# HKUST-KnowComp/DummyNode4GraphLearning

Hardware: AMD Instinct MI355X
Metric: edges/sec fwd+bwd on dummy-augmented RGIN conv (higher is better)
Workload: dtype bf16; 1 GPU; config5: RGINLayer(256,256,R=16,basis,relu) fwd+bwd, ONE global batch of 32768 graphs cut by parallel.shard_graphs over 1 GPU(s) (rank 0: N=1015808, E=3997696), SI dummy augmentation; global_edges=3997696, parallelism=dp1, rows_P=3112960, grad_bucket_bytes=2491904, hip_graph=True, sub_batches=1

## Files before the change

### dummynode4graphlearning_amd/csrc/dn_chain_wgrad.hip

```cpp
#include "dn_common.h"
#include "dn_internal.h"
#include "../../include/dn_hip.h"

namespace {

constexpr int kH = 256;
constexpr int kTile = 64;
constexpr int kKC = 32;
constexpr int kThreads = 256;
constexpr int kAld = kTile + 2;

__device__ __forceinline__ double bf16_to_f64(bf16_t v) { return (double)(float)v; }

__device__ __forceinline__ bf16_t f64_to_bf16(double d) {
    float f = (float)d;
    if ((double)f != d && f == f && fabsf(f) < __builtin_huge_valf()) {
        uint32_t u = __float_as_uint(f);
        if (fabs((double)f) > fabs(d)) u -= 1u;
        f = __uint_as_float(u | 1u);
    }
    return (bf16_t)f;
}

__global__ __launch_bounds__(kThreads) void chain_combine_products_kernel(const float* __restrict__ M, const bf16_t* __restrict__ W1,
                                                                          const bf16_t* __restrict__ Wc,
                                                                          const bf16_t* __restrict__ Wc_loop, int32_t R,
                                                                          bf16_t* __restrict__ dWc, double* __restrict__ part) {
    __shared__ __attribute__((aligned(16))) double As[kKC * kAld];
    __shared__ __attribute__((aligned(16))) double Bs[kKC * kTile];
    const int tid = threadIdx.x, ty = tid >> 4, tx = tid & 15;
    const int m0 = (int)(blockIdx.x >> 2) * kTile, n0 = (int)(blockIdx.x & 3) * kTile;
    const int r = (int)blockIdx.y, kind = (int)blockIdx.z;
    const float* Mr = M + (size_t)r * kH * kH;
    const bf16_t* B = kind == 0 ? W1 : (r < R ? Wc + (size_t)r * kH * kH : Wc_loop);
    double acc[4][4];
#pragma unroll
    for (int i = 0; i < 4; ++i)
#pragma unroll
        for (int j = 0; j < 4; ++j) acc[i][j] = 0.0;
    float ra[8];
    bf16_t rb[8];
    auto fetch = [&](int kc) __attribute__((always_inline)) {
#pragma unroll
        for (int s = 0; s < 8; ++s) {
            if (kind == 0) ra[s] = Mr[(size_t)(m0 + (tid >> 5) + 8 * s) * kH + kc + (tid & 31)];
            else ra[s] = Mr[(size_t)(kc + (tid >> 6) + 4 * s) * kH + m0 + (tid & 63)];
            rb[s] = B[(size_t)(kc + (tid >> 6) + 4 * s) * kH + n0 + (tid & 63)];
        }
    };
    fetch(0);
    for (int kc = 0; kc < kH; kc += kKC) {
#pragma unroll
        for (int s = 0; s < 8; ++s) {
            if (kind == 0) As[(tid & 31) * kAld + (tid >> 5) + 8 * s] = (double)ra[s];
            else As[((tid >> 6) + 4 * s) * kAld + (tid & 63)] = (double)ra[s];
            Bs[((tid >> 6) + 4 * s) * kTile + (tid & 63)] = bf16_to_f64(rb[s]);
        }
        if (kc + kKC < kH) fetch(kc + kKC);
        __syncthreads();
#pragma unroll 8
        for (int k = 0; k < kKC; ++k) {
            const double2 a01 = *reinterpret_cast<const double2*>(&As[k * kAld + 4 * ty]);
            const double2 a23 = *reinterpret_cast<const double2*>(&As[k * kAld + 4 * ty + 2]);
            const double2 b01 = *reinterpret_cast<const double2*>(&Bs[k * kTile + 4 * tx]);
            const double2 b23 = *reinterpret_cast<const double2*>(&Bs[k * kTile + 4 * tx + 2]);
            const double a[4] = {a01.x, a01.y, a23.x, a23.y}, b[4] = {b01.x, b01.y, b23.x, b23.y};
#pragma unroll
            for (int i = 0; i < 4; ++i)
#pragma unroll
                for (int j = 0; j < 4; ++j) acc[i][j] = fma(a[i], b[j], acc[i][j]);
        }
        __syncthreads();
    }
#pragma unroll
    for (int i = 0; i < 4; ++i)
#pragma unroll
        for (int j = 0; j < 4; ++j) {
            const size_t o = (size_t)r * kH * kH + (size_t)(m0 + 4 * ty + i) * kH + n0 + 4 * tx + j;
            if (kind == 0) dWc[o] = f64_to_bf16(acc[i][j]);
            else part[o] = acc[i][j];
        }
}

__global__ __launch_bounds__(kH) void chain_combine_finish_kernel(const double* __restrict__ part, const float* __restrict__ c,
                                                                  const bf16_t* __restrict__ W1, const bf16_t* __restrict__ bias,
                                                                  int32_t R, bf16_t* __restrict__ dW1, bf16_t* __restrict__ db,
                                                                  bf16_t* __restrict__ db1) {
    const int h = threadIdx.x, j = (int)blockIdx.x;
    if (j < kH) {
        double sum = 0.0;
        for (int r = 0; r <= R; ++r) sum += part[(size_t)r * kH * kH + (size_t)j * kH + h];
        if (bias) sum = fma((double)c[j], bf16_to_f64(bias[h]), sum);
        dW1[(size_t)j * kH + h] = f64_to_bf16(sum);
        return;
    }
    if (db) {
        double sum = 0.0;
        for (int jj = 0; jj < kH; ++jj) sum = fma((double)c[jj], bf16_to_f64(W1[(size_t)jj * kH + h]), sum);
        db[h] = f64_to_bf16(sum);
    }
    if (db1) db1[h] = (bf16_t)c[h];
}

}

extern "C" int dn_layer_chain_dgrad_bf16(const void* G1, const void* W_kn, int64_t N, int32_t H, const int32_t* tiles, int64_t num_tiles,
                                         void* G0, void* seg_sums, dn_stream_t stream) {
    DN_REQUIRE(H == 256, "dn_layer_chain_dgrad: unsupported width %d (256 only)", H);
    DN_REQUIRE(N >= 0 && N < 0x7fffffffLL && num_tiles >= 0 && num_tiles < 0x7fffffffLL, "dn_layer_chain_dgrad: bad sizes");
    if (num_tiles == 0) return DN_OK;
    DN_REQUIRE(G1 && W_kn && tiles && G0 && seg_sums, "dn_layer_chain_dgrad: NULL pointer");
    DN_REQUIRE((reinterpret_cast<uintptr_t>(G1) | reinterpret_cast<uintptr_t>(W_kn) | reinterpret_cast<uintptr_t>(tiles) |
                reinterpret_cast<uintptr_t>(G0) | reinterpret_cast<uintptr_t>(seg_sums)) % 16 == 0, "dn_layer_chain_dgrad: unaligned pointer");
    return dn_internal::launch_transform_ring256_seg(G1, W_kn, tiles, num_tiles, G0, seg_sums, (hipStream_t)stream);
}

extern "C" size_t dn_layer_chain_wgrad_combine_workspace_bytes(int64_t R, int32_t H) {
    return R >= 0 && H > 0 ? (size_t)(R + 1) * (size_t)H * (size_t)H * sizeof(double) : 0;
}

extern "C" int dn_layer_chain_wgrad_combine(const float* M, const float* c, const void* W1, const void* Wc, const void* Wc_loop,
                                            const void* bias, int64_t R, int32_t H, void* dWc, void* db, void* dW1, void* db1,
                                            void* workspace, size_t workspace_bytes, dn_stream_t stream) {
    DN_REQUIRE(H == 256, "dn_layer_chain_wgrad_combine: unsupported width %d (256 only)", H);
    DN_REQUIRE(R >= 0 && R < 65535, "dn_layer_chain_wgrad_combine: bad relation count");
    DN_REQUIRE(M && c && W1 && Wc_loop && dWc && dW1 && workspace && (Wc || R == 0), "dn_layer_chain_wgrad_combine: NULL pointer");
    DN_REQUIRE(workspace_bytes >= dn_layer_chain_wgrad_combine_workspace_bytes(R, H), "dn_layer_chain_wgrad_combine: workspace too small");
    DN_REQUIRE((reinterpret_cast<uintptr_t>(M) | reinterpret_cast<uintptr_t>(workspace)) % 16 == 0,
               "dn_layer_chain_wgrad_combine: unaligned pointer");
    hipStream_t st = (hipStream_t)stream;
    double* part = (double*)workspace;
    hipLaunchKernelGGL(chain_combine_products_kernel, dim3((kH / kTile) * (kH / kTile), (unsigned)(R + 1), 2), dim3(kThreads), 0, st, M,
                       (const bf16_t*)W1, (const bf16_t*)Wc, (const bf16_t*)Wc_loop, (int32_t)R, (bf16_t*)dWc, part);
    DN_CHECK_LAUNCH();
    hipLaunchKernelGGL(chain_combine_finish_kernel, dim3(kH + 1), dim3(kH), 0, st, (const double*)part, c, (const bf16_t*)W1,
                       (const bf16_t*)bias, (int32_t)R, (bf16_t*)dW1, (bf16_t*)db, (bf16_t*)db1);
    DN_CHECK_LAUNCH();
    return DN_OK;
}
```

Baseline: 1.430 billion edges/s.

## Rebalance wgrad combine GEMMs into persistent grid with tail slabs and double buffering

Replaces the per-tile 3D grid of fp64 combine GEMMs with a fixed persistent grid of 256 blocks. Each block runs larger 128x64 tiles, and the leftover tiles are split into small slabs spread across all blocks, so the last wave is not left lopsided. Shared-memory staging is double-buffered with register prefetch. The db/db1 reduction moves into an extra block of the products kernel, and the finish kernel batches its partial-sum loads. The trade-off is more register and LDS pressure per block and more complex scheduling code.

```diff
diff --git a/dummynode4graphlearning_amd/csrc/dn_chain_wgrad.hip b/dummynode4graphlearning_amd/csrc/dn_chain_wgrad.hip
--- a/dummynode4graphlearning_amd/csrc/dn_chain_wgrad.hip
+++ b/dummynode4graphlearning_amd/csrc/dn_chain_wgrad.hip
@@ -5,10 +5,14 @@
 namespace {
 
 constexpr int kH = 256;
-constexpr int kTile = 64;
-constexpr int kKC = 32;
+constexpr int kKC = 16;
+constexpr int kChunks = kH / kKC;
 constexpr int kThreads = 256;
-constexpr int kAld = kTile + 2;
+constexpr int kGrid = 256;
+constexpr int kAPad = 2;
+constexpr int kPartialBatch = 17;
+
+typedef double f64x2 __attribute__((ext_vector_type(2)));
 
 __device__ __forceinline__ double bf16_to_f64(bf16_t v) { return (double)(float)v; }
 
@@ -22,84 +26,212 @@
     return (bf16_t)f;
 }
 
-__global__ __launch_bounds__(kThreads) void chain_combine_products_kernel(const float* __restrict__ M, const bf16_t* __restrict__ W1,
-                                                                          const bf16_t* __restrict__ Wc,
-                                                                          const bf16_t* __restrict__ Wc_loop, int32_t R,
-                                                                          bf16_t* __restrict__ dWc, double* __restrict__ part) {
-    __shared__ __attribute__((aligned(16))) double As[kKC * kAld];
-    __shared__ __attribute__((aligned(16))) double Bs[kKC * kTile];
-    const int tid = threadIdx.x, ty = tid >> 4, tx = tid & 15;
-    const int m0 = (int)(blockIdx.x >> 2) * kTile, n0 = (int)(blockIdx.x & 3) * kTile;
-    const int r = (int)blockIdx.y, kind = (int)blockIdx.z;
-    const float* Mr = M + (size_t)r * kH * kH;
-    const bf16_t* B = kind == 0 ? W1 : (r < R ? Wc + (size_t)r * kH * kH : Wc_loop);
-    double acc[4][4];
-#pragma unroll
-    for (int i = 0; i < 4; ++i)
-#pragma unroll
-        for (int j = 0; j < 4; ++j) acc[i][j] = 0.0;
-    float ra[8];
-    bf16_t rb[8];
-    auto fetch = [&](int kc) __attribute__((always_inline)) {
-#pragma unroll
-        for (int s = 0; s < 8; ++s) {
-            if (kind == 0) ra[s] = Mr[(size_t)(m0 + (tid >> 5) + 8 * s) * kH + kc + (tid & 31)];
-            else ra[s] = Mr[(size_t)(kc + (tid >> 6) + 4 * s) * kH + m0 + (tid & 63)];
-            rb[s] = B[(size_t)(kc + (tid >> 6) + 4 * s) * kH + n0 + (tid & 63)];
-        }
+template <int TX, int RPT, int NP>
+struct CombineJob {
+    static constexpr int TM = (kThreads / TX) * RPT, TN = 2 * TX * NP, ALD = TM + kAPad;
+    static constexpr int NA = TM * kKC / kThreads, NB = kKC * TN / kThreads;
+    static constexpr int kStageA = kKC * ALD, kStageB = kKC * TN;
+    static_assert(TM * kKC % kThreads == 0 && kKC * TN % kThreads == 0 && (RPT == 1 || RPT % 2 == 0) && (TM & (TM - 1)) == 0, "job shape");
+    const float* Mr;
+    const bf16_t* B;
+    bf16_t* out_bf16;
+    double* out_f64;
+    double* As;
+    double* Bs;
+    int kind, m0, n0;
+    double acc[RPT][2 * NP];
+    float ra[NA];
+    bf16_t rb[NB];
+
+    __device__ __forceinline__ void zero() {
+#pragma unroll
+        for (int i = 0; i < RPT; ++i)
+#pragma unroll
+            for (int j = 0; j < 2 * NP; ++j) acc[i][j] = 0.0;
+    }
+    __device__ __forceinline__ void fetch(int kc) {
+        const int tid = threadIdx.x;
+        const float* a = kind == 0 ? Mr + (size_t)(m0 + tid / kKC) * kH + kc + tid % kKC : Mr + (size_t)(kc + tid / TM) * kH + m0 + tid % TM;
+        const int a_step = kind == 0 ? (kThreads / kKC) * kH : (kThreads / TM) * kH;
+#pragma unroll
+        for (int s = 0; s < NA; ++s) ra[s] = a[s * a_step];
+#pragma unroll
+        for (int s = 0; s < NB; ++s) {
+            const int e = tid + kThreads * s;
+            rb[s] = B[(size_t)(kc + e / TN) * kH + n0 + e % TN];
+        }
+    }
+    __device__ __forceinline__ void stage(int st) {
+        const int tid = threadIdx.x;
+        double* a = As + st * kStageA + (kind == 0 ? (tid % kKC) * ALD + tid / kKC : (tid / TM) * ALD + tid % TM);
+        const int a_step = kind == 0 ? kThreads / kKC : (kThreads / TM) * ALD;
+        double* b = Bs + st * kStageB;
+#pragma unroll
+        for (int s = 0; s < NA; ++s) a[s * a_step] = (double)ra[s];
+#pragma unroll
+        for (int s = 0; s < NB; ++s) b[tid + kThreads * s] = bf16_to_f64(rb[s]);
+    }
+    struct Operands {
+        double a[RPT], b[2 * NP];
     };
-    fetch(0);
-    for (int kc = 0; kc < kH; kc += kKC) {
-#pragma unroll
-        for (int s = 0; s < 8; ++s) {
-            if (kind == 0) As[(tid & 31) * kAld + (tid >> 5) + 8 * s] = (double)ra[s];
-            else As[((tid >> 6) + 4 * s) * kAld + (tid & 63)] = (double)ra[s];
-            Bs[((tid >> 6) + 4 * s) * kTile + (tid & 63)] = bf16_to_f64(rb[s]);
-        }
-        if (kc + kKC < kH) fetch(kc + kKC);
+    __device__ __forceinline__ void load(int st, int k, Operands& o) const {
+        const int ty = threadIdx.x / TX, tx = threadIdx.x % TX;
+        const double* a_s = As + st * kStageA + k * ALD + RPT * ty;
+        const double* b_s = Bs + st * kStageB + k * TN + 2 * tx;
+        if constexpr (RPT == 1) {
+            o.a[0] = a_s[0];
+        } else {
+#pragma unroll
+            for (int i = 0; i < RPT; i += 2) {
+                const f64x2 v = *reinterpret_cast<const f64x2*>(&a_s[i]);
+                o.a[i] = v.x;
+                o.a[i + 1] = v.y;
+            }
+        }
+#pragma unroll
+        for (int q = 0; q < NP; ++q) {
+            const f64x2 v = *reinterpret_cast<const f64x2*>(&b_s[2 * TX * q]);
+            o.b[2 * q] = v.x;
+            o.b[2 * q + 1] = v.y;
+        }
+    }
+    __device__ __forceinline__ void fmas(const Operands& o) {
+#pragma unroll
+        for (int i = 0; i < RPT; ++i)
+#pragma unroll
+            for (int j = 0; j < 2 * NP; ++j) acc[i][j] = fma(o.a[i], o.b[j], acc[i][j]);
+    }
+    __device__ __forceinline__ void store() const {
+        const int ty = threadIdx.x / TX, tx = threadIdx.x % TX;
+#pragma unroll
+        for (int i = 0; i < RPT; ++i)
+#pragma unroll
+            for (int j = 0; j < 2 * NP; ++j) {
+                const size_t o = (size_t)(m0 + RPT * ty + i) * kH + n0 + 2 * TX * (j / 2) + 2 * tx + j % 2;
+                if (kind == 0) out_bf16[o] = f64_to_bf16(acc[i][j]);
+                else out_f64[o] = acc[i][j];
+            }
+    }
+};
+
+using TileJob = CombineJob<16, 8, 2>;
+using SlabJob = CombineJob<16, 1, 1>;
+constexpr int kTileCols = kH / TileJob::TN;
+constexpr int kTilesPerProduct = (kH / TileJob::TM) * kTileCols;
+constexpr int kSlabCols = TileJob::TN / SlabJob::TN;
+constexpr int kSlabsPerTile = (TileJob::TM / SlabJob::TM) * kSlabCols;
+
+template <bool T, bool S>
+__device__ __forceinline__ void combine_run(TileJob& t, SlabJob& s) {
+    if (T) t.zero(), t.fetch(0), t.stage(0);
+    if (S) s.zero(), s.fetch(0), s.stage(0);
+    __syncthreads();
+    for (int c = 0; c < kChunks; ++c) {
+        const bool more = c + 1 < kChunks;
+        if (more) {
+            if (T) t.fetch((c + 1) * kKC);
+            if (S) s.fetch((c + 1) * kKC);
+        }
+        TileJob::Operands t0, t1;
+        SlabJob::Operands s0, s1;
+        const int st = c & 1;
+        auto load = [&](int k, TileJob::Operands& to, SlabJob::Operands& so) __attribute__((always_inline)) {
+            if (T) t.load(st, k, to);
+            if (S) s.load(st, k, so);
+        };
+        auto fmas = [&](const TileJob::Operands& to, const SlabJob::Operands& so) __attribute__((always_inline)) {
+            if (T) t.fmas(to);
+            if (S) s.fmas(so);
+        };
+        load(0, t0, s0);
+#pragma unroll 1
+        for (int k = 0; k < kKC - 2; k += 2) {
+            load(k + 1, t1, s1);
+            fmas(t0, s0);
+            load(k + 2, t0, s0);
+            fmas(t1, s1);
+        }
+        load(kKC - 1, t1, s1);
+        fmas(t0, s0);
+        fmas(t1, s1);
+        if (more) {
+            if (T) t.stage((c + 1) & 1);
+            if (S) s.stage((c + 1) & 1);
+        }
         __syncthreads();
-#pragma unroll 8
-        for (int k = 0; k < kKC; ++k) {
-            const double2 a01 = *reinterpret_cast<const double2*>(&As[k * kAld + 4 * ty]);
-            const double2 a23 = *reinterpret_cast<const double2*>(&As[k * kAld + 4 * ty + 2]);
-            const double2 b01 = *reinterpret_cast<const double2*>(&Bs[k * kTile + 4 * tx]);
-            const double2 b23 = *reinterpret_cast<const double2*>(&Bs[k * kTile + 4 * tx + 2]);
-            const double a[4] = {a01.x, a01.y, a23.x, a23.y}, b[4] = {b01.x, b01.y, b23.x, b23.y};
-#pragma unroll
-            for (int i = 0; i < 4; ++i)
-#pragma unroll
-                for (int j = 0; j < 4; ++j) acc[i][j] = fma(a[i], b[j], acc[i][j]);
-        }
-        __syncthreads();
-    }
-#pragma unroll
-    for (int i = 0; i < 4; ++i)
-#pragma unroll
-        for (int j = 0; j < 4; ++j) {
-            const size_t o = (size_t)r * kH * kH + (size_t)(m0 + 4 * ty + i) * kH + n0 + 4 * tx + j;
-            if (kind == 0) dWc[o] = f64_to_bf16(acc[i][j]);
-            else part[o] = acc[i][j];
-        }
+    }
+    if (T) t.store();
+    if (S) s.store();
+}
+
+__global__ __launch_bounds__(kThreads, 2) void chain_combine_products_kernel(const float* __restrict__ M, const bf16_t* __restrict__ W1,
+                                                                             const bf16_t* __restrict__ Wc,
+                                                                             const bf16_t* __restrict__ Wc_loop, int32_t R,
+                                                                             bf16_t* __restrict__ dWc, double* __restrict__ part,
+                                                                             const float* __restrict__ c, bf16_t* __restrict__ db,
+                                                                             bf16_t* __restrict__ db1) {
+    __shared__ __attribute__((aligned(16))) double At[2 * TileJob::kStageA];
+    __shared__ __attribute__((aligned(16))) double Bt[2 * TileJob::kStageB];
+    __shared__ __attribute__((aligned(16))) double As[2 * SlabJob::kStageA];
+    __shared__ __attribute__((aligned(16))) double Bs[2 * SlabJob::kStageB];
+    constexpr int G = kGrid;
+    const int w = (int)blockIdx.x;
+    if (w == G) {
+        const int h = threadIdx.x;
+        if (db) {
+            double sum = 0.0;
+#pragma unroll 32
+            for (int j = 0; j < kH; ++j) sum = fma((double)c[j], bf16_to_f64(W1[(size_t)j * kH + h]), sum);
+            db[h] = f64_to_bf16(sum);
+        }
+        if (db1) db1[h] = (bf16_t)c[h];
+        return;
+    }
+    const int tiles = 2 * (R + 1) * kTilesPerProduct;
+    const int whole = tiles / G * G;
+    const int slabs = (tiles - whole) * kSlabsPerTile;
+    TileJob t;
+    SlabJob s;
+    t.As = At, t.Bs = Bt, s.As = As, s.Bs = Bs;
+    auto place = [&](auto& job, int tile, int dm, int dn) __attribute__((always_inline)) {
+        const int p = tile / kTilesPerProduct, q = tile % kTilesPerProduct;
+        const int r = p % (R + 1);
+        const size_t base = (size_t)r * kH * kH;
+        job.kind = p / (R + 1);
+        job.m0 = (q / kTileCols) * TileJob::TM + dm;
+        job.n0 = (q % kTileCols) * TileJob::TN + dn;
+        job.Mr = M + base;
+        job.B = job.kind == 0 ? W1 : (r < R ? Wc + base : Wc_loop);
+        job.out_bf16 = dWc + base;
+        job.out_f64 = part + base;
+    };
+    for (int i = 0;; ++i) {
+        const int tile = w + i * G, slab = w + i * G;
+        const bool ht = tile < whole, hs = slab < slabs;
+        if (!ht && !hs) break;
+        if (ht) place(t, tile, 0, 0);
+        if (hs) place(s, whole + slab / kSlabsPerTile, (slab % kSlabsPerTile / kSlabCols) * SlabJob::TM, (slab % kSlabCols) * SlabJob::TN);
+        if (ht && hs) combine_run<true, true>(t, s);
+        else if (ht) combine_run<true, false>(t, s);
+        else combine_run<false, true>(t, s);
+    }
 }
 
 __global__ __launch_bounds__(kH) void chain_combine_finish_kernel(const double* __restrict__ part, const float* __restrict__ c,
-                                                                  const bf16_t* __restrict__ W1, const bf16_t* __restrict__ bias,
-                                                                  int32_t R, bf16_t* __restrict__ dW1, bf16_t* __restrict__ db,
-                                                                  bf16_t* __restrict__ db1) {
+                                                                  const bf16_t* __restrict__ bias, int32_t R, bf16_t* __restrict__ dW1) {
     const int h = threadIdx.x, j = (int)blockIdx.x;
-    if (j < kH) {
-        double sum = 0.0;
-        for (int r = 0; r <= R; ++r) sum += part[(size_t)r * kH * kH + (size_t)j * kH + h];
-        if (bias) sum = fma((double)c[j], bf16_to_f64(bias[h]), sum);
-        dW1[(size_t)j * kH + h] = f64_to_bf16(sum);
-        return;
-    }
-    if (db) {
-        double sum = 0.0;
-        for (int jj = 0; jj < kH; ++jj) sum = fma((double)c[jj], bf16_to_f64(W1[(size_t)jj * kH + h]), sum);
-        db[h] = f64_to_bf16(sum);
-    }
-    if (db1) db1[h] = (bf16_t)c[h];
+    const double* p = part + (size_t)j * kH + h;
+    double sum = 0.0;
+    for (int r0 = 0; r0 <= R; r0 += kPartialBatch) {
+        double v[kPartialBatch];
+#pragma unroll
+        for (int i = 0; i < kPartialBatch; ++i) v[i] = r0 + i <= R ? p[(size_t)(r0 + i) * kH * kH] : 0.0;
+#pragma unroll
+        for (int i = 0; i < kPartialBatch; ++i)
+            if (r0 + i <= R) sum += v[i];
+    }
+    if (bias) sum = fma((double)c[j], bf16_to_f64(bias[h]), sum);
+    dW1[(size_t)j * kH + h] = f64_to_bf16(sum);
 }
 
 }
@@ -130,11 +262,11 @@
                "dn_layer_chain_wgrad_combine: unaligned pointer");
     hipStream_t st = (hipStream_t)stream;
     double* part = (double*)workspace;
-    hipLaunchKernelGGL(chain_combine_products_kernel, dim3((kH / kTile) * (kH / kTile), (unsigned)(R + 1), 2), dim3(kThreads), 0, st, M,
-                       (const bf16_t*)W1, (const bf16_t*)Wc, (const bf16_t*)Wc_loop, (int32_t)R, (bf16_t*)dWc, part);
+    hipLaunchKernelGGL(chain_combine_products_kernel, dim3(kGrid + 1), dim3(kThreads), 0, st, M, (const bf16_t*)W1, (const bf16_t*)Wc,
+                       (const bf16_t*)Wc_loop, (int32_t)R, (bf16_t*)dWc, part, c, (bf16_t*)db, (bf16_t*)db1);
     DN_CHECK_LAUNCH();
-    hipLaunchKernelGGL(chain_combine_finish_kernel, dim3(kH + 1), dim3(kH), 0, st, (const double*)part, c, (const bf16_t*)W1,
-                       (const bf16_t*)bias, (int32_t)R, (bf16_t*)dW1, (bf16_t*)db, (bf16_t*)db1);
+    hipLaunchKernelGGL(chain_combine_finish_kernel, dim3(kH), dim3(kH), 0, st, (const double*)part, c, (const bf16_t*)bias, (int32_t)R,
+                       (bf16_t*)dW1);
     DN_CHECK_LAUNCH();
     return DN_OK;
 }
```

New measurement: 1.438 billion edges/s, median of 6. No clear change (+0.5%).
